# lixinghe1999/VRVQ

Measured on AMD Instinct MI355X. Metric: audio-sec/s encode+RVQ+decode, 44.1 kHz batch-32, 1->8 MI355X; RVQ HBM GB/s, higher is better.
Workload: dtype f32; 1 GPU; DAC_VRVQ VBR 8 cb, level 1.0, 1-s clips, preprocess+encode+decode (z_q_is materialised); model=DAC_VRVQ base (8 cb), global_batch=32, clip_samples=44100, n_codebooks=8, parallelism=dp1 (replicas, no data-path collective)

## Files before the change

include/vrvq.h:

```cpp
#ifndef VRVQ_H_
#define VRVQ_H_

#include <stdint.h>

#ifdef __cplusplus
extern "C" {
#endif

typedef void* vrvq_stream_t;

enum vrvq_status_t {
  VRVQ_OK = 0,
  VRVQ_ERR_ARG = 10001,
  VRVQ_ERR_UNSUPPORTED = 10002
};

enum vrvq_epilogue_t { VRVQ_EPI_NONE = 0, VRVQ_EPI_TANH = 1, VRVQ_EPI_SIGMOID = 2 };

const char* vrvq_status_string(int status);
int vrvq_version(void);


int vrvq_weight_norm(const float* g, const float* v, int rows, int cols, float* w,
                     vrvq_stream_t stream);
// ... 21 lines not shown
                          int dil, int x3, long long* bytes);
int vrvq_conv1d_ws(const float* x, int batch, int cin, int tin, const float* alpha,
                   const float* inv_alpha, const float* w_packed, const uint16_t* w_x3, int cout,
                   int cout_pad, int k, int stride, int pad, int dil, const float* bias,
                   const float* residual, int epilogue, float* y, int tout,
                   const float* alpha_out, const float* inv_alpha_out, float* y_snake,
                   void* workspace, long long ws_bytes, vrvq_stream_t stream);

int vrvq_x3_weight_size(int cin, int k, int cout_pad, long long* n_u16);
int vrvq_pack_x3_weight(const float* w_packed, int cin, int k, int cout_pad, uint16_t* w_x3,
                        vrvq_stream_t stream);

int vrvq_conv1d_proj(const float* x, int batch, int cin, int tin, const float* alpha,
                     const float* inv_alpha, const float* w_packed, const uint16_t* w_x3, int cout,
                     int cout_pad, int k, int pad, int dil, const float* bias, float* y, int tout,
                     const uint16_t* w3in, int nq, float* part, void* workspace,
                     long long ws_bytes, vrvq_stream_t stream);

int vrvq_conv_last_launch(int out[5]);

enum vrvq_plan_kind_t { VRVQ_PLAN_CONV = 0, VRVQ_PLAN_PROJ = 1, VRVQ_PLAN_CONV_TRANSPOSE = 2 };
int vrvq_conv_plan(int kind, int batch, int cin, int tin, int cout, int k, int stride, int pad,
                   int dil, int has_x3, int has_workspace, int out[7]);

int vrvq_pack_conv1d_weight(const float* w, int cout, int cin, int k, int cout_pad,
                            float* w_packed, vrvq_stream_t stream);

int vrvq_residual_unit(const float* x, const float* x_snk, int batch, int channels, int frames,
                       int dil, const float* w7_packed, const uint16_t* w7_x3,
                       const uint16_t* w1_x3, const float* b7,
                       const float* alpha2,
                       const float* inv_alpha2, const float* w1_packed, const float* b1,
                       int cout_pad, float* y, const float* alpha_out,
                       const float* inv_alpha_out, float* y_snake, vrvq_stream_t stream);

int vrvq_conv_transpose1d(const float* x, int batch, int cin, int tin, const float* alpha,
                          const float* inv_alpha, const float* w_packed, int cout,
                          int cout_pad, int stride, const float* bias, float* y,
                          const float* alpha_out, const float* inv_alpha_out, float* y_snake,
                          vrvq_stream_t stream);

int vrvq_conv_transpose1d_pad(const float* x, int batch, int cin, int tin, const float* alpha,
                              const float* inv_alpha, const float* w_packed,
                              const uint16_t* w_x3, int cout,
                              int cout_pad, int stride, int pad, const float* bias, float* y,
                              const float* alpha_out, const float* inv_alpha_out,
// ... 235 lines not shown
```

vrvq_amd/_lib.py:

```python
from __future__ import annotations

import ctypes
import os
import threading

LIB_NAME = "libvrvq_hip.so"
LIB_PATH = os.environ.get("VRVQ_LIB") or os.path.join(os.path.dirname(os.path.abspath(__file__)), LIB_NAME)

_P = ctypes.c_void_p
_I = ctypes.c_int
_F = ctypes.c_float

SIGNATURES = {
    "vrvq_weight_norm": [_P, _P, _I, _I, _P, _P],
    "vrvq_snake_inv_alpha": [_P, _I, _P, _P],
    "vrvq_snake": [_P, _I, _I, _I, _P, _P, _P, _P],
    "vrvq_phase_split": [_P, _I, _I, _I, _I, _I, _I, _P, _P, _P, _P],
    "vrvq_codebook_prep": [_P, _I, _I, _P, _P, _P],
    "vrvq_conv1d": [_P, _I, _I, _I, _P, _P, _P, _P, _I, _I, _I, _I, _I, _I, _P, _P, _I, _P, _I,
                    _P, _P, _P, _P],
    "vrvq_conv1d_workspace": [_I, _I, _I, _I, _I, _I, _I, _I, _I, _P],
    "vrvq_conv1d_ws": [_P, _I, _I, _I, _P, _P, _P, _P, _I, _I, _I, _I, _I, _I, _P, _P, _I, _P,
                       _I, _P, _P, _P, _P, ctypes.c_longlong, _P],
    "vrvq_conv1d_proj": [_P, _I, _I, _I, _P, _P, _P, _P, _I, _I, _I, _I, _I, _P, _P, _I, _P, _I,
                         _P, _P, ctypes.c_longlong, _P],
    "vrvq_x3_weight_size": [_I, _I, _I, _P],
    "vrvq_pack_x3_weight": [_P, _I, _I, _I, _P, _P],
    "vrvq_pack_conv1d_weight": [_P, _I, _I, _I, _I, _P, _P],
    "vrvq_residual_unit": [_P, _P, _I, _I, _I, _I, _P, _P, _P, _P, _P, _P, _P, _P, _I, _P, _P,
                           _P, _P, _P],
    "vrvq_conv_transpose1d": [_P, _I, _I, _I, _P, _P, _P, _I, _I, _I, _P, _P, _P, _P, _P, _P],
    "vrvq_conv_transpose1d_pad": [_P, _I, _I, _I, _P, _P, _P, _P, _I, _I, _I, _I, _P, _P, _P, _P,
                                  _P, _P],
    "vrvq_pack_convt1d_weight": [_P, _I, _I, _I, _I, _P, _P],
    "vrvq_rvq_cross_prep": [_P, _P, _P, _I, _I, _I, _P, _P, _P],
    "vrvq_rvq_frag": [_P, _I, _I, _I, _P, _P],
    "vrvq_rvq_workspace": [_I, _I, _I, _P],
    "vrvq_rvq_encode": [_P, _I, _I, _I, _I, _I, _I, _P, _P, _P, _P, _P, _P, _P, _P, _P, _P, _F,
                        _P, _P, _P, _P, _P, _P, _P, ctypes.c_longlong, _P],
    "vrvq_rvq_w_in_planes_size": [_I, _I, _I, _P],
    "vrvq_rvq_pack_w_in": [_P, _I, _I, _I, _P, _P],
    "vrvq_rvq_workspace_part": [_I, _I, _I, _I, _P],
    "vrvq_rvq_encode_part": [_P, _I, _I, _I, _I, _I, _I, _P, _P, _P, _P, _P, _P, _P, _P, _P, _F,
                             _P, _P, _P, _P, _P, _P, _P, ctypes.c_longlong, _P],
    "vrvq_rvq_fused_clips": [_I, _I, _I, _P],
    "vrvq_rvq_project": [_P, _I, _I, _I, _I, _I, _P, _P, _P],
    "vrvq_rvq_chain": [_P, _I, _I, _I, _I, _I, _P, _P, _P, _P, _P, _P, _P, _F, _P, _P, _P, _P, _P,
                       _P],
# ... 44 lines not shown
    "vrvq_conv1d_wgrad": [_P, _I, _I, _I, _P, _P, _P, _I, _I, _P, _P, _I, _I, _I, _I, _I, _P,
                          ctypes.c_longlong, _P, _P],
    "vrvq_snake_backward_workspace": [_I, _I, _I, _P],
    "vrvq_snake_backward": [_P, _P, _P, _P, _I, _I, _I, _P, _P, _P, ctypes.c_longlong, _P],
    "vrvq_bias_grad_workspace": [_I, _I, _I, _P],
    "vrvq_bias_grad": [_P, _I, _I, _I, _P, _P, ctypes.c_longlong, _P],
    "vrvq_act_backward": [_P, _P, ctypes.c_longlong, _I, _P, _P],
    "vrvq_weight_norm_backward": [_P, _P, _P, _I, _I, _P, _P, _P],
    "vrvq_pack_conv1d_flip": [_P, _I, _I, _I, _I, _P, _P],
    "vrvq_mask_ste": [_P, _P, _P, _I, _I, _I, _F, _I, _I, _P, _P],
    "vrvq_mask_ste_backward": [_P, _P, _P, _I, _I, _I, _F, _I, _P, _P],
    "vrvq_rvq_expand_masked": [_P, _I, _I, _I, _I, _I, _P, _P, _P, _P, _P, _P],
    "vrvq_rvq_backward_workspace": [_I, _I, _I, _P],
    "vrvq_rvq_backward": [_P, _P, _P, _P, _P, _P, _P, _P, _I, _I, _I, _I, _I, _I, _P, _P, _P,
                          _P, _P, _P, _P, _P, _P, _P, _P, _P, _P, ctypes.c_longlong, _P],
}
EXTRA = {"vrvq_status_string": ([_I], ctypes.c_char_p), "vrvq_version": ([], _I),
         "vrvq_rvq_path": ([_I], _I), "vrvq_rvq_plan": ([_I] * 5 + [_P], _I),
         "vrvq_rvq_sync_error": ([_P, _P], _I), "vrvq_rvq_timing": ([_I], _I),
         "vrvq_rvq_timing_read": ([_P, _P], _I), "vrvq_rvq_pending_error": ([_P], _I),
         "vrvq_rvq_debug": ([ctypes.c_uint, ctypes.c_uint], _I),
         "vrvq_rvq_debug_capacity": ([_I], _I), "vrvq_conv_last_launch": ([_P], _I),
         "vrvq_conv_plan": ([_I] * 11 + [_P], _I),
         "vrvq_resample_error": ([], ctypes.c_char_p),
         "vrvq_loudness_error": ([], ctypes.c_char_p),
         "vrvq_bitstream_chunk_frames": ([], _I)}

METRICS_CHUNK = 16384
SPECTRAL_TILE_SAMPLES = 8192
RESAMPLE_TILE = 512
LOUDNESS_CHUNK = 256
LOUDNESS_PLAN_LEN = 30
BITSTREAM_CHUNK_FRAMES = 256


def spectral_tile_frames(window: int) -> int:
    return SPECTRAL_TILE_SAMPLES // int(window)

_lock = threading.Lock()
_lib = None


def load() -> ctypes.CDLL:
    global _lib
    if _lib is not None:
        return _lib
# ... 55 lines not shown


def rvq_debug_capacity(clips: int) -> int:
    return int(load().vrvq_rvq_debug_capacity(int(clips)))


def conv_last_launch() -> dict:
    out = (ctypes.c_int * 5)()
    call("vrvq_conv_last_launch", out)
    return dict(zip(("BM", "BN", "KS", "x3", "S"), (int(v) for v in out)))


PLAN_KINDS = {"conv": 0, "proj": 1, "convt": 2}


def conv_plan(kind, batch: int, cin: int, tin: int, cout: int, k: int, stride: int = 1,
              pad: int = 0, dil: int = 1, x3: bool = True, workspace: bool = True) -> dict:
    out = (ctypes.c_int * 7)()
    call("vrvq_conv_plan", PLAN_KINDS.get(kind, kind), batch, cin, tin, cout, k, stride, pad, dil,
         1 if x3 else 0, 1 if workspace else 0, out)
    return dict(zip(("BM", "BN", "KS", "x3", "S", "path", "WM"), (int(v) for v in out)))


def rvq_timing(on: bool) -> bool:
    return bool(load().vrvq_rvq_timing(1 if on else 0))


def rvq_timing_read():
    ms, n = ctypes.c_float(0.0), ctypes.c_int(0)
    call("vrvq_rvq_timing_read", ctypes.byref(ms), ctypes.byref(n))
    return float(ms.value), int(n.value)


RVQ_PLAN_KEYS = ("kind", "F", "P", "n_fb", "wg_per_clip", "lds", "resident", "clips", "launches",
                 "ws_bytes")
RVQ_PLAN_PT, RVQ_PLAN_CHAIN_EXPAND = 0, 1


def rvq_plan(batch: int, frames: int, nq: int, ncode: int = 1024, resident: int = 0) -> dict:
    out = (ctypes.c_longlong * 10)()
    call("vrvq_rvq_plan", batch, frames, nq, ncode, resident, out)
    return dict(zip(RVQ_PLAN_KEYS, (int(v) for v in out)))


RESAMPLE_PLAN_KEYS = ("old", "new", "W", "K", "ntaps", "out_length", "out_length_max",
                      "taps_len")
# ... 52 lines not shown
```

vrvq_amd/csrc/conv_geom.h:

```cpp
#pragma once

namespace vrvq_conv {

constexpr int chunk_ck(int ks, int bm, int bn) {
  const int ck0 = ks == 1 ? 32 : ks <= 3 ? 16 : ks == 4 ? 8 : ks == 7 ? 8
                  : ks == 8 ? 4 : bn > 32 ? 4 : 2;
  return (bm > 128 && ck0 >= 8) ? ck0 / 2 : ck0;
}

constexpr int win_smax(int ks) { return (ks == 4 || ks == 8 || ks == 16) ? ks / 2 : 1; }
constexpr int win_dmax(int ks) { return ks == 7 ? 9 : 1; }
constexpr int win_xw_max(int ks, int bn) {
  return (bn - 1) * win_smax(ks) + (ks - 1) * win_dmax(ks) + 1;
}
constexpr int win_per_row(int ks, int bn) { return (win_xw_max(ks, bn) + 63) / 64; }

constexpr long long conv_lds_bytes(int ks, int bm, int bn, int xwp) {
  const long long ck = chunk_ck(ks, bm, bn);
  return 2 * (ck * ks * bm + ck * xwp) * 4;
}

constexpr int epi_passes(int bm, int bn) {
  const int need = (bm * bn * 4 + 65535) / 65536;
  return need <= 1 ? 1 : need <= 2 ? 2 : need <= 4 ? 4 : 8;
// ... 16 lines not shown
}
constexpr int x3_nc8(int ks, bool pair) { return x3_ck(ks, pair) / 8; }
constexpr int x3_no(int ks, bool pair) { return ks * x3_nc8(ks, pair); }
constexpr int x3_no2(int ks, bool pair) { return (x3_no(ks, pair) + 1) & ~1; }
constexpr int x3_nstep(int ks, bool pair) { return x3_no2(ks, pair) / 2; }

constexpr int x3_xw_max(int ks, int bn) { return (bn - 1) + (ks - 1) * (ks == 7 ? 9 : 1) + 1; }
constexpr int x3_xwp(int xw) { return (xw + 3) & ~3; }

constexpr int x3_stage_w_bytes(int ks, int bm, bool pair) {
  return pair ? 2 * 3 * x3_no(ks, false) * bm * 16 : 3 * x3_no2(ks, false) * bm * 16;
}

constexpr long long x3_lds_bytes(int ks, int bm, int bn, bool pair, int xw, int snake_cin) {
  const long long xb = 3LL * x3_nc8(ks, pair) * x3_xwp(xw) * 16;
  const long long snake = pair ? 2LL * snake_cin * 4 : 0;
  return x3_stages(bm, bn) * (x3_stage_w_bytes(ks, bm, pair) + xb) + snake;
}

constexpr bool x3_offsets_fit(long long tin, long long m_pad) {
  return 32 * tin * 4 <= 0x7fffffffLL && 49 * m_pad * 16 <= 0x7fffffffLL;
}

constexpr int SMALL_BT = 256;
constexpr int SMALL_SC = 16;
constexpr int SMALL_COUT = 8;
constexpr int SMALL_WMAX = 2048;
constexpr int C1_T = 4;
constexpr int C1_W = 12;
constexpr int CI1_T = 4;
constexpr int CI1_CG = 16;

}
```

vrvq_amd/csrc/misc.hip:

```cpp
#include "common.h"

namespace {

__global__ __launch_bounds__(256) void weight_norm_kernel(const float* __restrict__ g,
                                                          const float* __restrict__ v, int cols,
                                                          float* __restrict__ w) {
  __shared__ float part[256];
  const size_t row = blockIdx.x;
  const float* vr = v + row * cols;
  float ss = 0.0f;
  for (int c = threadIdx.x; c < cols; c += 256) ss = fmaf(vr[c], vr[c], ss);
  part[threadIdx.x] = ss;
  __syncthreads();
  for (int h = 128; h >= 1; h >>= 1) {
    if ((int)threadIdx.x < h) part[threadIdx.x] += part[threadIdx.x + h];
    __syncthreads();
  }
  const float scale = g[row] / sqrtf(part[0]);
  for (int c = threadIdx.x; c < cols; c += 256) w[row * cols + c] = vr[c] * scale;
}

__global__ void inv_alpha_kernel(const float* __restrict__ alpha, int n, float* __restrict__ inv) {
  const int i = blockIdx.x * blockDim.x + threadIdx.x;
  if (i < n) inv[i] = 1.0f / (alpha[i] + 1e-9f);
// ... 193 lines not shown
  if (cdim != 8 || ncode > 4096) return VRVQ_ERR_UNSUPPORTED;
  const long long nf = (long long)batch * frames;
  VRVQ_CHECK_ARG((nf + 255) / 256 < 0x7fffffffLL);
  const size_t lds = (size_t)ncode * 9 * sizeof(float);
  if (lds > 64 * 1024) {
    hipError_t e = hipFuncSetAttribute((const void*)rvq_nearest_kernel,
                                       hipFuncAttributeMaxDynamicSharedMemorySize, (int)lds);
    if (e != hipSuccess) return (int)e;
  }
  hipLaunchKernelGGL(rvq_nearest_kernel, dim3((unsigned)((nf + 255) / 256), nq), dim3(256), lds,
                     as_stream(stream), latents, batch, nlat, frames, cbn, c2, ncode, codes, nq);
  return vrvq_launch_status();
}

extern "C" const char* vrvq_status_string(int status) {
  switch (status) {
    case VRVQ_OK: return "ok";
    case VRVQ_ERR_ARG: return "vrvq: invalid argument (null pointer, size or shape mismatch)";
    case VRVQ_ERR_UNSUPPORTED: return "vrvq: shape outside the instantiated kernel set";
    default: return hipGetErrorString((hipError_t)status);
  }
}

extern "C" int vrvq_version(void) { return 111; }

extern "C" int vrvq_weight_norm(const float* g, const float* v, int rows, int cols, float* w,
                                vrvq_stream_t stream) {
  VRVQ_CHECK_ARG(g && v && w && rows > 0 && cols > 0);
  hipLaunchKernelGGL(weight_norm_kernel, dim3(rows), dim3(256), 0, as_stream(stream), g, v, cols, w);
  return vrvq_launch_status();
}

__global__ __launch_bounds__(256) void snake_rows_kernel(const float* __restrict__ x,
                                                         const float* __restrict__ alpha,
                                                         const float* __restrict__ inv_alpha,
                                                         int channels, int frames, int nseg,
                                                         float* __restrict__ y) {
  const int row = blockIdx.x / nseg, seg = blockIdx.x - row * nseg;
  const int c = row % channels;
  const float al = alpha[c], ia = inv_alpha[c];
  const size_t base = (size_t)row * frames;
#pragma unroll
  for (int u = 0; u < 4; ++u) {
    const int t = seg * 1024 + u * 256 + (int)threadIdx.x;
    if (t < frames) y[base + t] = snake_act(x[base + t], al, ia);
  }
}
// ... 118 lines not shown
```

vrvq_amd/csrc/torch_ops.cpp:

```cpp
#include <ATen/core/Tensor.h>
#include <ATen/ops/empty.h>
#include <ATen/ops/empty_like.h>
#include <ATen/ops/zeros.h>
#include <c10/core/DeviceGuard.h>
#include <c10/hip/HIPStream.h>
#include <torch/library.h>

#include <vector>

#include "../../include/vrvq.h"

namespace {

using at::Tensor;
using c10::optional;

void* stream_of(const Tensor& t) {
  return reinterpret_cast<void*>(c10::hip::getCurrentHIPStream(t.device().index()).stream());
}

void check_rc(int rc, const char* fn) {
  TORCH_CHECK(rc == 0, fn, " failed (", rc, "): ", vrvq_status_string(rc));
}

// ... 157 lines not shown
  TORCH_CHECK(alpha.has_value() == inv_alpha.has_value(), "conv1d: snake needs inv_alpha");
  c10::DeviceGuard guard(x.device());
  const int64_t k = w_packed.size(1), cout_pad = w_packed.size(2);
  const int64_t tout = (tin + 2 * pad - dil * (k - 1) - 1) / stride + 1;
  TORCH_CHECK(tout > 0, "conv1d: input too short");
  if (residual.has_value())
    TORCH_CHECK(residual->sizes() == at::IntArrayRef({B, cout, tout}),
                "conv1d: residual shape must equal the output shape");
  auto [y, ys, _u] = out_pair(x, {B, cout, tout}, alpha_out, inv_alpha_out, want_raw);
  const uint16_t* w3 = stride > 1 ? x3_ptr(w_x3, x, cin * stride, 2, cout_pad)
                                  : x3_ptr(w_x3, x, cin, k, cout_pad);
  long long ws_bytes = 0;
  check_rc(vrvq_conv1d_workspace((int)B, (int)cin, (int)tin, (int)cout, (int)k, (int)stride,
                                 (int)pad, (int)dil, w3 != nullptr, &ws_bytes),
           "vrvq_conv1d_workspace");
  Tensor ws = ws_bytes > 0 ? at::empty({(ws_bytes + 3) / 4}, x.options()) : Tensor();
  check_rc(vrvq_conv1d_ws(x.data_ptr<float>(), (int)B, (int)cin, (int)tin, fp(alpha),
                          fp(inv_alpha), w_packed.data_ptr<float>(), w3, (int)cout,
                          (int)cout_pad, (int)k, (int)stride, (int)pad, (int)dil, fp(bias),
                          fp(residual), (int)epilogue, y.numel() ? y.data_ptr<float>() : nullptr,
                          (int)tout, fp(alpha_out), fp(inv_alpha_out), opt_ptr(ys),
                          ws_bytes > 0 ? ws.data_ptr() : nullptr, ws_bytes, stream_of(x)),
           "vrvq_conv1d_ws");
  return {y, ys};
}

std::tuple<Tensor, Tensor> snake_conv_transpose1d(
    const Tensor& x, const Tensor& w_packed, int64_t cout, int64_t stride,
    const optional<Tensor>& bias, const optional<Tensor>& alpha,
    const optional<Tensor>& inv_alpha, const optional<Tensor>& alpha_out,
    const optional<Tensor>& inv_alpha_out, bool want_raw, int64_t pad,
    const optional<Tensor>& w_x3) {
  check_t(x, "x");
  check_on(w_packed, x, "w_packed");
  check_opt(bias, x, "bias");
  check_opt(alpha, x, "alpha");
  check_opt(inv_alpha, x, "inv_alpha");
  TORCH_CHECK(x.dim() == 3, "conv_transpose1d: x must be (B, C, T)");
  const int64_t p = pad < 0 ? (stride + 1) / 2 : pad;
  TORCH_CHECK(p < stride, "conv_transpose1d: padding must be < stride");
  TORCH_CHECK(w_packed.dim() == 3 && w_packed.size(0) == x.size(1) && w_packed.size(1) == 2,
              "conv_transpose1d: w_packed must be (Cin, 2, cout_pad)");
  TORCH_CHECK(alpha.has_value() == inv_alpha.has_value(),
              "conv_transpose1d: snake needs inv_alpha");
  c10::DeviceGuard guard(x.device());
  const int64_t B = x.size(0), cin = x.size(1), tin = x.size(2);
// ... 1195 lines not shown
  Tensor ws = at::empty({ws_doubles}, x.options().dtype(at::kDouble));
  Tensor out = at::empty({items}, x.options().dtype(at::kDouble));
  check_rc(vrvq_loudness(x.data_ptr<float>(), (int)items, (int)nch, L, (int)sample_rate,
                         ws.data_ptr<double>(), out.data_ptr<double>(), stream_of(x)),
           "vrvq_loudness");
  return out;
}

}

TORCH_LIBRARY(vrvq, m) {
  m.def("weight_norm(Tensor g, Tensor v) -> Tensor");
  m.def("snake_inv_alpha(Tensor alpha) -> Tensor");
  m.def("codebook_prep(Tensor cb) -> (Tensor, Tensor)");
  m.def("pack_conv1d_weight(Tensor w) -> Tensor");
  m.def("pack_convt1d_weight(Tensor w, int stride) -> Tensor");
  m.def("pack_x3_weight(Tensor w_packed, int k) -> Tensor");
  m.def(
      "snake_conv1d(Tensor x, Tensor w_packed, int cout, int stride, int pad, int dil, "
      "Tensor? bias, Tensor? alpha, Tensor? inv_alpha, Tensor? residual, int epilogue, "
      "Tensor? alpha_out, Tensor? inv_alpha_out, bool want_raw, Tensor? w_x3=None) "
      "-> (Tensor, Tensor)");
  m.def(
      "snake_conv_transpose1d(Tensor x, Tensor w_packed, int cout, int stride, Tensor? bias, "
      "Tensor? alpha, Tensor? inv_alpha, Tensor? alpha_out, Tensor? inv_alpha_out, "
      "bool want_raw, int pad=-1, Tensor? w_x3=None) -> (Tensor, Tensor)");
  m.def(
      "residual_unit(Tensor x, Tensor x_snk, int dil, Tensor w7, Tensor b7, Tensor alpha2, "
      "Tensor inv_alpha2, Tensor w1, Tensor b1, Tensor? alpha_out, Tensor? inv_alpha_out, "
      "bool want_raw, Tensor? w7_x3=None, Tensor? w1_x3=None) -> (Tensor, Tensor)");
  m.def("rvq_cross_prep(Tensor w_in_t, Tensor w_out, Tensor b_out) -> (Tensor, Tensor)");
  m.def("rvq_frag(Tensor cbn) -> Tensor");
  m.def(
      "rvq_encode(Tensor z, Tensor w_in_t, Tensor b_in, Tensor cb, Tensor cbf, Tensor c2, "
      "Tensor w_out, Tensor b_out, Tensor mcol, Tensor qb, Tensor? imp, float level, "
      "bool want_z_q_is, bool want_mask) -> (Tensor, Tensor, Tensor, Tensor, Tensor, Tensor)");
  m.def("rvq_pack_w_in(Tensor w_in_t) -> Tensor");
  m.def(
      "snake_conv1d_proj(Tensor x, Tensor w_packed, int cout, int pad, int dil, Tensor? bias, "
      "Tensor? alpha, Tensor? inv_alpha, Tensor? w_x3, Tensor w3in, int nq, bool want_z) "
      "-> (Tensor, Tensor)");
  m.def(
      "rvq_encode_part(Tensor part, int frames, Tensor b_in, Tensor cb, Tensor cbf, Tensor c2, "
      "Tensor w_out, Tensor b_out, Tensor mcol, Tensor qb, Tensor? imp, float level, "
      "bool want_z_q_is, bool want_mask) -> (Tensor, Tensor, Tensor, Tensor, Tensor, Tensor)");
  m.def("rvq_check_error(Tensor like, bool sync) -> int");
// ... 67 lines not shown
      "Tensor w_out, Tensor b_out, Tensor mcol, Tensor qb, Tensor mask) "
      "-> (Tensor, Tensor, Tensor, Tensor, Tensor)");
  m.def(
      "rvq_backward(Tensor dz_q, Tensor g_commit, Tensor g_codebook, Tensor z, Tensor zst, "
      "Tensor latents, Tensor codes, Tensor mask, Tensor w_in_t, Tensor w_out, Tensor b_out, "
      "Tensor mcol, Tensor cb) -> (Tensor, Tensor, Tensor, Tensor, Tensor, Tensor, Tensor)");
  m.def(
      "resample(Tensor x, Tensor taps, Tensor first, int old_rate, int width, int out_length) "
      "-> Tensor");
  m.def(
      "resample_adjoint(Tensor dy, Tensor taps, Tensor first, int old_rate, int width, "
      "int length) -> Tensor");
  m.def("loudness(Tensor x, int sample_rate) -> Tensor");
}

#define VRVQ_IMPLS(m) \
  m.impl("weight_norm", &weight_norm); \
  m.impl("snake_inv_alpha", &snake_inv_alpha); \
  m.impl("codebook_prep", &codebook_prep); \
  m.impl("pack_conv1d_weight", &pack_conv1d_weight); \
  m.impl("pack_convt1d_weight", &pack_convt1d_weight); \
  m.impl("pack_x3_weight", &pack_x3_weight); \
  m.impl("snake_conv1d", &snake_conv1d); \
  m.impl("snake_conv_transpose1d", &snake_conv_transpose1d); \
  m.impl("residual_unit", &residual_unit); \
  m.impl("rvq_cross_prep", &rvq_cross_prep); \
  m.impl("rvq_frag", &rvq_frag); \
  m.impl("rvq_encode", &rvq_encode); \
  m.impl("rvq_pack_w_in", &rvq_pack_w_in); \
  m.impl("snake_conv1d_proj", &snake_conv1d_proj); \
  m.impl("rvq_encode_part", &rvq_encode_part); \
  m.impl("rvq_check_error", &rvq_check_error); \
  m.impl("rvq_gather", &rvq_gather); \
  m.impl("rvq_nearest", &rvq_nearest); \
  m.impl("rvq_expand", &rvq_expand); \
  m.impl("masked_loss", &masked_loss); \
  m.impl("scale_imp", &scale_imp); \
  m.impl("imp_mask", &imp_mask); \
  m.impl("masked_sum", &masked_sum); \
  m.impl("bpf", &bpf); \
  m.impl("rate_curve", &rate_curve); \
  m.impl("rate_solve", &rate_solve); \
  m.impl("scale_imp_rows", &scale_imp_rows); \
  m.impl("rate_solve_capped", &rate_solve_capped); \
  m.impl("scale_imp_packets", &scale_imp_packets); \
  m.impl("signal_metrics", &signal_metrics); \
// ... 28 lines not shown
```

vrvq_amd/layers.py:

```python
from __future__ import annotations

import math
from typing import Optional

import torch
import torch.nn as nn

from . import ops


def _param_key(*ps):
    return tuple((p.device, p.data_ptr(), p._version) for p in ps)


class Snake1d(nn.Module):

    def __init__(self, channels: int):
        super().__init__()
        self.channels = channels
        self.alpha = nn.Parameter(torch.ones(1, channels, 1))
        self._cache = None

    def prepared(self):
        key = _param_key(self.alpha)
# ... 161 lines not shown
            x = x[..., pad:-pad].contiguous()
        return self.block[3](y, snake=self.block[2], residual=x)

    def runs_fused(self) -> bool:
        C = self.block[1].in_channels
        return self.fused and C in ops.RU_FUSED_CHANNELS and not (C == 256 and ops.X3 and
                                                                 ops.RU256_SPLIT)

    def run(self, x: torch.Tensor, x_snk: torch.Tensor, out_snake: Snake1d, want_raw: bool):
        if self.runs_fused():
            w7, cp7 = self.block[1].prepared()
            w1, cp1 = self.block[3].prepared()
            a2, ia2 = self.block[2].prepared()
            return ops.residual_unit(x, x_snk, self.block[1].dilation[0], w7,
                                     self.block[1].bias.detach(), a2, ia2, w1,
                                     self.block[3].bias.detach(), cp7,
                                     out_snake=out_snake.prepared(), want_raw=want_raw,
                                     w7_x3=self.block[1].prepared_x3(),
                                     w1_x3=self.block[3].prepared_x3())
        return self.run_two_launch(x, x_snk, out_snake, want_raw)

    def run_two_launch(self, x, x_snk, out_snake: Snake1d, want_raw: bool):
        _, h_snk = self.block[1](x_snk, out_snake=self.block[2], want_raw=False)
        return self.block[3](h_snk, residual=x, out_snake=out_snake, want_raw=want_raw)


class EncoderBlock(nn.Module):

    def __init__(self, dim: int = 16, stride: int = 1):
        super().__init__()
        self.block = nn.Sequential(
            ResidualUnit(dim // 2, dilation=1),
            ResidualUnit(dim // 2, dilation=3),
            ResidualUnit(dim // 2, dilation=9),
            Snake1d(dim // 2),
            WNConv1d(dim // 2, dim, kernel_size=2 * stride, stride=stride,
                     padding=math.ceil(stride / 2)),
        )

    def forward(self, x):
        for i in range(3):
            x = self.block[i](x)
        return self.block[4](x, snake=self.block[3])

    def entry_snake(self) -> Snake1d:
        return self.block[0].block[0]

# ... 38 lines not shown
```

vrvq_amd/ops.py:

```python
from __future__ import annotations

import os
import threading
from typing import Optional, Tuple

import torch

EPI_NONE, EPI_TANH, EPI_SIGMOID = 0, 1, 2

_HERE = os.path.dirname(os.path.abspath(__file__))
TORCH_LIB_PATH = os.environ.get("VRVQ_TORCH_LIB") or os.path.join(_HERE, "libvrvq_torch.so")
_lock = threading.Lock()
_loaded = False


def load_ops():
    global _loaded
    if _loaded:
        return torch.ops.vrvq
    with _lock:
        if not _loaded:
            if not os.path.exists(TORCH_LIB_PATH):
                raise RuntimeError(
                    f"vrvq_amd: operator library {TORCH_LIB_PATH} is missing; build it with "
# ... 46 lines not shown
    return wp, wp.shape[2]


def pack_convt1d_weight(w: torch.Tensor, stride: int) -> Tuple[torch.Tensor, int]:
    wp = _ops().pack_convt1d_weight(w, int(stride))
    return wp, wp.shape[2]


def conv1d(x: torch.Tensor, w_packed: torch.Tensor, cout: int, cout_pad: int, k: int,
           stride: int = 1, pad: int = 0, dil: int = 1, bias: Optional[torch.Tensor] = None,
           alpha: Optional[torch.Tensor] = None, inv_alpha: Optional[torch.Tensor] = None,
           residual: Optional[torch.Tensor] = None, epilogue: int = EPI_NONE,
           out_snake: Optional[Tuple[torch.Tensor, torch.Tensor]] = None, want_raw: bool = True,
           w_x3: Optional[torch.Tensor] = None):
    if w_packed.dim() != 3 or w_packed.shape[1] != k or w_packed.shape[2] != cout_pad:
        raise RuntimeError("conv1d: w_packed must be (Cin, k, cout_pad)")
    ao, io = out_snake if out_snake is not None else (None, None)
    y, ys = _ops().snake_conv1d(x, w_packed, int(cout), int(stride), int(pad), int(dil), bias,
                                alpha, inv_alpha, residual, int(epilogue), ao, io, bool(want_raw),
                                w_x3)
    return _none(y) if out_snake is None else (_none(y), ys)


def conv1d_proj(x: torch.Tensor, w_packed: torch.Tensor, cout: int, k: int, w3in: torch.Tensor,
                nq: int, pad: int = 0, dil: int = 1, bias: Optional[torch.Tensor] = None,
                alpha: Optional[torch.Tensor] = None, inv_alpha: Optional[torch.Tensor] = None,
                w_x3: Optional[torch.Tensor] = None, want_z: bool = False):
    if w_packed.dim() != 3 or w_packed.shape[1] != k:
        raise RuntimeError("conv1d_proj: w_packed must be (Cin, k, cout_pad)")
    part, z = _ops().snake_conv1d_proj(x, w_packed, int(cout), int(pad), int(dil), bias, alpha,
                                       inv_alpha, w_x3, w3in, int(nq), bool(want_z))
    return part, _none(z)


def conv_transpose1d(x: torch.Tensor, w_packed: torch.Tensor, cout: int, cout_pad: int,
                     stride: int, bias: Optional[torch.Tensor] = None,
                     alpha: Optional[torch.Tensor] = None,
                     inv_alpha: Optional[torch.Tensor] = None,
                     out_snake: Optional[Tuple[torch.Tensor, torch.Tensor]] = None,
                     want_raw: bool = True, pad: int = -1,
                     w_x3: Optional[torch.Tensor] = None):
    ao, io = out_snake if out_snake is not None else (None, None)
    y, ys = _ops().snake_conv_transpose1d(x, w_packed, int(cout), int(stride), bias, alpha,
                                          inv_alpha, ao, io, bool(want_raw), int(pad), w_x3)
    return _none(y) if out_snake is None else (_none(y), ys)

# ... 247 lines not shown

    @reg("vrvq::pack_x3_weight")
    def _(w_packed, k):
        cin, _k, cout_pad = w_packed.shape
        return torch.empty(x3_size(cin, k, cout_pad), dtype=torch.int16, device=w_packed.device)

    @reg("vrvq::pack_convt1d_weight")
    def _(w, stride):
        cin, cout, _k = w.shape
        return f32(w, (cin, 2, round_up(cout * stride, 128 if 128 % stride == 0 else 192)))

    def pair(x, shape, ao, want_raw):
        ys = f32(x, shape) if ao is not None else none(x)
        y = f32(x, shape) if (want_raw or ao is None) else none(x)
        return y, ys

    @reg("vrvq::snake_conv1d")
    def _(x, w_packed, cout, stride, pad, dil, bias, alpha, inv_alpha, residual, epilogue,
          alpha_out, inv_alpha_out, want_raw, w_x3=None):
        B, _c, tin = x.shape
        tout = conv_out_len(tin, w_packed.shape[1], stride, pad, dil)
        return pair(x, (B, cout, tout), alpha_out, want_raw)

    @reg("vrvq::snake_conv_transpose1d")
    def _(x, w_packed, cout, stride, bias, alpha, inv_alpha, alpha_out, inv_alpha_out, want_raw,
          pad=-1, w_x3=None):
        B, _c, tin = x.shape
        tout = convt_out_len(tin, stride, pad)
        return pair(x, (B, cout, tout), alpha_out, want_raw)

    @reg("vrvq::residual_unit")
    def _(x, x_snk, dil, w7, b7, alpha2, inv_alpha2, w1, b1, alpha_out, inv_alpha_out, want_raw,
          w7_x3=None, w1_x3=None):
        return pair(x, tuple(x.shape), alpha_out, want_raw)

    @reg("vrvq::rvq_cross_prep")
    def _(w_in_t, w_out, b_out):
        nq, _D, d = w_in_t.shape
        return f32(w_in_t, (nq, nq, d, d)), f32(w_in_t, (nq, d))

    @reg("vrvq::rvq_frag")
    def _(cbn):
        return torch.empty_like(cbn)

    @reg("vrvq::rvq_encode")
    def _(z, w_in_t, b_in, cb, cbf, c2, w_out, b_out, mcol, qb, imp, level, want_z_q_is,
# ... 219 lines not shown
```

Baseline: 806.6 audio-sec/s.

## Add specialized k=1 conv kernel with fused residual and snake for residual units

Adds a dedicated pointwise (k=1) convolution kernel for the residual-unit second conv. It stages the whole input-channel slice in LDS as three bf16 split planes, runs the x3 bf16 MFMA accumulation with double-buffered weight loads, and fuses bias, residual add and the output snake into the epilogue. Residual loads are issued early to overlap with staging. It replaces the generic conv path in run_two_launch when the channel count is 192/256/384, falling back otherwise. It costs extra code paths and large LDS use, which may reduce occupancy.

New measurement: 811.8 audio-sec/s, median of 6. Within noise of the previous version (+0.6%).

```diff
diff --git a/include/vrvq.h b/include/vrvq.h
--- a/include/vrvq.h
+++ b/include/vrvq.h
@@ -67,6 +67,12 @@
 enum vrvq_plan_kind_t { VRVQ_PLAN_CONV = 0, VRVQ_PLAN_PROJ = 1, VRVQ_PLAN_CONV_TRANSPOSE = 2 };
 int vrvq_conv_plan(int kind, int batch, int cin, int tin, int cout, int k, int stride, int pad,
                    int dil, int has_x3, int has_workspace, int out[7]);
+
+int vrvq_conv1d_k1_skip(const float* x, int batch, int cin, int tin, const uint16_t* w_x3,
+                        int cout, int cout_pad, const float* bias, const float* residual,
+                        float* y, const float* alpha_out, const float* inv_alpha_out,
+                        float* y_snake, vrvq_stream_t stream);
+int vrvq_conv1d_k1_skip_plan(int batch, int cin, int tin, int cout, int out[5]);
 
 int vrvq_pack_conv1d_weight(const float* w, int cout, int cin, int k, int cout_pad,
                             float* w_packed, vrvq_stream_t stream);
diff --git a/vrvq_amd/_lib.py b/vrvq_amd/_lib.py
--- a/vrvq_amd/_lib.py
+++ b/vrvq_amd/_lib.py
@@ -24,6 +24,7 @@
                        _I, _P, _P, _P, _P, ctypes.c_longlong, _P],
     "vrvq_conv1d_proj": [_P, _I, _I, _I, _P, _P, _P, _P, _I, _I, _I, _I, _I, _P, _P, _I, _P, _I,
                          _P, _P, ctypes.c_longlong, _P],
+    "vrvq_conv1d_k1_skip": [_P, _I, _I, _I, _P, _I, _I, _P, _P, _P, _P, _P, _P, _P],
     "vrvq_x3_weight_size": [_I, _I, _I, _P],
     "vrvq_pack_x3_weight": [_P, _I, _I, _I, _P, _P],
     "vrvq_pack_conv1d_weight": [_P, _I, _I, _I, _I, _P, _P],
@@ -114,6 +115,7 @@
          "vrvq_rvq_debug": ([ctypes.c_uint, ctypes.c_uint], _I),
          "vrvq_rvq_debug_capacity": ([_I], _I), "vrvq_conv_last_launch": ([_P], _I),
          "vrvq_conv_plan": ([_I] * 11 + [_P], _I),
+         "vrvq_conv1d_k1_skip_plan": ([_I] * 4 + [_P], _I),
          "vrvq_resample_error": ([], ctypes.c_char_p),
          "vrvq_loudness_error": ([], ctypes.c_char_p),
          "vrvq_bitstream_chunk_frames": ([], _I)}
@@ -215,6 +217,24 @@
     return dict(zip(("BM", "BN", "KS", "x3", "S", "path", "WM"), (int(v) for v in out)))
 
 
+K1_SKIP_PLAN_KEYS = ("BM", "BN", "threads", "lds", "grid")
+ERR_UNSUPPORTED = 10002
+
+
+def k1_skip_plan(batch: int, channels: int, frames: int, cout: int = 0):
+    out = (ctypes.c_int * 5)()
+    lib = load()
+    rc = lib.vrvq_conv1d_k1_skip_plan(int(batch), int(channels), int(frames),
+                                      int(cout or channels), out)
+    if rc == ERR_UNSUPPORTED:
+        return None
+    if rc != 0:
+        msg = lib.vrvq_status_string(rc)
+        raise RuntimeError(f"vrvq_conv1d_k1_skip_plan failed ({rc}): "
+                           f"{msg.decode() if msg else 'unknown'}")
+    return dict(zip(K1_SKIP_PLAN_KEYS, (int(v) for v in out)))
+
+
 def rvq_timing(on: bool) -> bool:
     return bool(load().vrvq_rvq_timing(1 if on else 0))
 
diff --git a/vrvq_amd/csrc/conv_geom.h b/vrvq_amd/csrc/conv_geom.h
--- a/vrvq_amd/csrc/conv_geom.h
+++ b/vrvq_amd/csrc/conv_geom.h
@@ -62,6 +62,23 @@
   return 32 * tin * 4 <= 0x7fffffffLL && 49 * m_pad * 16 <= 0x7fffffffLL;
 }
 
+struct K1sTile {
+  int BM, BN, WM, NW, WPE;
+};
+constexpr K1sTile k1s_tile(int c) {
+  return c == 192 ? K1sTile{192, 64, 2, 4, 2}
+       : c == 256 ? K1sTile{256, 64, 4, 8, 2}
+       : c == 384 ? K1sTile{384, 64, 4, 8, 2}
+                  : K1sTile{0, 0, 0, 0, 0};
+}
+constexpr long long k1s_lds_bytes(int c, int bn) { return 6LL * c * bn; }
+constexpr long long k1s_lds_total(int c, int bm, int bn) { return k1s_lds_bytes(c, bn) + 3LL * bm * 4; }
+constexpr bool k1s_offsets_fit(long long c, long long tin) { return c * tin * 4 <= 0x7fffffffLL; }
+constexpr long long k1s_grid(int c, long long batch, long long tin) {
+  const K1sTile t = k1s_tile(c);
+  return t.BM == 0 ? 0 : batch * ((tin + t.BN - 1) / t.BN) * (c / t.BM);
+}
+
 constexpr int SMALL_BT = 256;
 constexpr int SMALL_SC = 16;
 constexpr int SMALL_COUT = 8;
diff --git a/vrvq_amd/csrc/conv_k1_skip.hip b/vrvq_amd/csrc/conv_k1_skip.hip
--- /dev/null
+++ b/vrvq_amd/csrc/conv_k1_skip.hip
@@ -0,0 +1,271 @@
+#include "common.h"
+#include "conv_core.h"
+#include "conv_x3.h"
+
+namespace {
+
+using namespace vrvq_conv;
+
+struct K1sArgs {
+  const float* x;
+  const u32x4* w3;
+  const float* bias;
+  const float* res;
+  float* y;
+  const float* alpha_o;
+  const float* inv_alpha_o;
+  float* ys;
+  int tin, m_pad, n_nt;
+};
+
+typedef float f32x4u __attribute__((ext_vector_type(4), aligned(4)));
+
+template <int C, int BM, int BN, int WM, int NW, int WPE>
+__global__ __launch_bounds__(64 * NW) __attribute__((amdgpu_waves_per_eu(WPE, WPE)))
+void k1_skip_kernel(K1sArgs a) {
+  using TC = TileCfg<BM, BN, WM, NW>;
+  constexpr int NT = TC::NT, RM = TC::RM, RN = TC::RN, TM = TC::TM, TN = TC::TN;
+  constexpr int NC8 = C / 8;
+  constexpr int NQ = C / 16;
+  constexpr int N_MT = C / BM;
+  constexpr int XI = NC8 * BN / NT;
+  constexpr int NV = BN / 4;
+  constexpr int ITER = BM * NV / NT;
+  static_assert(C % 32 == 0 && C % BM == 0, "whole k = 1 chunks, whole row tiles");
+  static_assert((NC8 * BN) % NT == 0 && NT % BN == 0, "staging: whole items, one column per thread");
+  static_assert((BM * NV) % NT == 0 && NT % NV == 0, "epilogue: whole items, one column group per thread");
+  static_assert(RM >= 1 && RN >= 1 && TM % 32 == 0 && TN % 32 == 0 && NQ % 2 == 0, "tile");
+  extern __shared__ __attribute__((aligned(16))) float smem[];
+
+  int blk = blockIdx.x;
+  const int m0 = (blk % N_MT) * BM;
+  blk /= N_MT;
+  const int nt = blk % a.n_nt, b = blk / a.n_nt;
+  const int n0 = nt * BN;
+  const int T = a.tin;
+  const int tid = threadIdx.x, lane = tid & 63, wave = tid >> 6;
+  const int wm = wave % WM, wn = wave / WM;
+  const int lr = lane & 31, lh = lane >> 5;
+
+  float* tab = reinterpret_cast<float*>(reinterpret_cast<char*>(smem) + k1s_lds_bytes(C, BN));
+  for (int r = tid; r < BM; r += NT) {
+    tab[r] = a.bias ? a.bias[m0 + r] : 0.0f;
+    tab[BM + r] = a.ys ? a.alpha_o[m0 + r] : 0.0f;
+    tab[2 * BM + r] = a.ys ? a.inv_alpha_o[m0 + r] : 0.0f;
+  }
+
+  const int ncols = min(BN, T - n0);
+  const int nl = (tid % NV) * 4;
+  const bool inrow = nl + 4 <= ncols;
+  f32x4u rs[ITER];
+  {
+    const float* xb = a.x + (size_t)b * C * T;
+    const int col = tid % BN, t = n0 + col;
+    const unsigned xo = ((unsigned)((tid / BN) * 8) * (unsigned)T + (unsigned)min(t, T - 1)) * 4u;
+    float xr[XI][8];
+#pragma unroll
+    for (int it = 0; it < XI; ++it)
+#pragma unroll
+      for (int u = 0; u < 8; ++u) {
+        const float* xu = xb + (size_t)(it * (NT / BN) * 8 + u) * T;
+        xr[it][u] = *reinterpret_cast<const float*>(reinterpret_cast<const char*>(xu) + xo);
+      }
+    __builtin_amdgcn_sched_barrier(0);
+    {
+      const float* resb = a.res + (size_t)b * C * T;
+      const unsigned ro = inrow ? ((unsigned)(m0 + tid / NV) * (unsigned)T + (unsigned)(n0 + nl)) * 4u : 0u;
+      const unsigned rstep = inrow ? (unsigned)(NT / NV) * (unsigned)T * 4u : 0u;
+#pragma unroll
+      for (int it = 0; it < ITER; ++it)
+        rs[it] = *reinterpret_cast<const f32x4u*>(reinterpret_cast<const char*>(resb) + (ro + it * rstep));
+    }
+    __builtin_amdgcn_sched_barrier(0);
+    u32x4* xs = reinterpret_cast<u32x4*>(smem);
+    const bool ok = t < T;
+#pragma unroll
+    for (int it = 0; it < XI; ++it) {
+      float v[8];
+#pragma unroll
+      for (int u = 0; u < 8; ++u) v[u] = ok ? xr[it][u] : 0.0f;
+      unsigned h[4], m[4], l[4];
+#pragma unroll
+      for (int u = 0; u < 4; ++u) split3x2(v[2 * u], v[2 * u + 1], h[u], m[u], l[u]);
+      const int e = tid + it * NT;
+      xs[0 * NC8 * BN + e] = u32x4{h[0], h[1], h[2], h[3]};
+      xs[1 * NC8 * BN + e] = u32x4{m[0], m[1], m[2], m[3]};
+      xs[2 * NC8 * BN + e] = u32x4{l[0], l[1], l[2], l[3]};
+    }
+  }
+  __syncthreads();
+
+  f32x16 acc[RM][RN];
+#pragma unroll
+  for (int i = 0; i < RM; ++i)
+#pragma unroll
+    for (int j = 0; j < RN; ++j)
+#pragma unroll
+      for (int r = 0; r < 16; ++r) acc[i][j][r] = 0.0f;
+
+  const u32x4* hs = reinterpret_cast<const u32x4*>(smem);
+  const unsigned wlo = ((unsigned)lh * (unsigned)a.m_pad + (unsigned)(m0 + wm * TM + lr)) * 16u;
+  auto lda = [&](int q, u32x4 (&av)[3][RM]) {
+    const u32x4* wq = a.w3 + (size_t)((q >> 1) * 12 + 2 * (q & 1)) * a.m_pad;
+    const unsigned wl = x3_opaque(wlo);
+#pragma unroll
+    for (int p = 0; p < 3; ++p)
+#pragma unroll
+      for (int i = 0; i < RM; ++i)
+        av[p][i] = *reinterpret_cast<const u32x4*>(
+            reinterpret_cast<const char*>(wq + (size_t)(p * 4) * a.m_pad + i * 32) + wl);
+  };
+  auto step = [&](int q, const u32x4 (&av)[3][RM]) {
+    u32x4 bv[3][RN];
+    const int o = 2 * q + lh;
+#pragma unroll
+    for (int p = 0; p < 3; ++p)
+#pragma unroll
+      for (int j = 0; j < RN; ++j) bv[p][j] = hs[((size_t)p * NC8 + o) * BN + wn * TN + j * 32 + lr];
+#pragma unroll
+    for (int i = 0; i < RM; ++i)
+#pragma unroll
+      for (int j = 0; j < RN; ++j) {
+        f32x16 t = acc[i][j];
+        t = mfma_bf16(av[1][i], bv[1][j], t);
+        t = mfma_bf16(av[0][i], bv[2][j], t);
+        t = mfma_bf16(av[2][i], bv[0][j], t);
+        t = mfma_bf16(av[0][i], bv[1][j], t);
+        t = mfma_bf16(av[1][i], bv[0][j], t);
+        acc[i][j] = mfma_bf16(av[0][i], bv[0][j], t);
+      }
+  };
+  u32x4 a0[3][RM], a1[3][RM];
+  lda(0, a0);
+#pragma unroll 1
+  for (int q = 0; q < NQ; q += 2) {
+    lda(q + 1, a1);
+    __builtin_amdgcn_sched_barrier(0);
+    step(q, a0);
+    __builtin_amdgcn_sched_barrier(0);
+    lda(min(q + 2, NQ - 1), a0);
+    __builtin_amdgcn_sched_barrier(0);
+    step(q + 1, a1);
+    __builtin_amdgcn_sched_barrier(0);
+  }
+  __syncthreads();
+
+  float* ct = smem;
+#pragma unroll
+  for (int i = 0; i < RM; ++i)
+#pragma unroll
+    for (int j = 0; j < RN; ++j)
+#pragma unroll
+      for (int r = 0; r < 16; ++r)
+        ct[(wm * TM + i * 32 + (r & 3) + 8 * (r >> 2) + 4 * lh) * BN + wn * TN + j * 32 + lr] =
+            acc[i][j][r];
+  __syncthreads();
+  if (ncols == BN && (T & 3) == 0) {
+#pragma unroll
+    for (int it = 0; it < ITER; ++it) {
+      const int ml = tid / NV + it * (NT / NV);
+      const float4 c = *reinterpret_cast<const float4*>(ct + ml * BN + nl);
+      const float bb = tab[ml];
+      float v[4] = {c.x + bb, c.y + bb, c.z + bb, c.w + bb};
+#pragma unroll
+      for (int q = 0; q < 4; ++q) v[q] = rs[it][q] + v[q];
+      const size_t ob = ((size_t)b * C + m0 + ml) * T + n0 + nl;
+      if (a.y) *reinterpret_cast<float4*>(a.y + ob) = make_float4(v[0], v[1], v[2], v[3]);
+      if (a.ys) {
+        snake_n1<4>(v, tab[BM + ml], tab[2 * BM + ml]);
+        *reinterpret_cast<float4*>(a.ys + ob) = make_float4(v[0], v[1], v[2], v[3]);
+      }
+    }
+    return;
+  }
+  if (nl >= ncols) return;
+#pragma unroll 1
+  for (int it = 0; it < ITER; ++it) {
+    const int ml = tid / NV + it * (NT / NV);
+    const float4 c = *reinterpret_cast<const float4*>(ct + ml * BN + nl);
+    const float bb = tab[ml];
+    float v[4] = {c.x + bb, c.y + bb, c.z + bb, c.w + bb};
+    const size_t ob = ((size_t)b * C + m0 + ml) * T + n0 + nl;
+#pragma unroll
+    for (int q = 0; q < 4; ++q)
+      if (nl + q < ncols) v[q] = a.res[ob + q] + v[q];
+    if (a.y) {
+#pragma unroll
+      for (int q = 0; q < 4; ++q)
+        if (nl + q < ncols) a.y[ob + q] = v[q];
+    }
+    if (a.ys) {
+      snake_n1<4>(v, tab[BM + ml], tab[2 * BM + ml]);
+#pragma unroll
+      for (int q = 0; q < 4; ++q)
+        if (nl + q < ncols) a.ys[ob + q] = v[q];
+    }
+  }
+}
+
+template <int C>
+int launch_k1s(K1sArgs a, int batch, hipStream_t st) {
+  constexpr K1sTile t = k1s_tile(C);
+  static_assert(t.BM > 0, "no tile for this C");
+  constexpr int lds = (int)k1s_lds_total(C, t.BM, t.BN);
+  static_assert(lds <= 160 * 1024, "planes fit in LDS");
+  auto kernel = k1_skip_kernel<C, t.BM, t.BN, t.WM, t.NW, t.WPE>;
+  const long long grid = k1s_grid(C, batch, a.tin);
+  if (grid <= 0 || grid > 0x7fffffffLL) return VRVQ_ERR_ARG;
+  a.n_nt = (a.tin + t.BN - 1) / t.BN;
+  if (lds > 64 * 1024) {
+    hipError_t e = hipFuncSetAttribute((const void*)kernel,
+                                       hipFuncAttributeMaxDynamicSharedMemorySize, lds);
+    if (e != hipSuccess) return (int)e;
+  }
+  hipLaunchKernelGGL(kernel, dim3((unsigned)grid), dim3(64 * t.NW), lds, st, a);
+  return vrvq_launch_status();
+}
+
+bool k1s_geometry_ok(int batch, int cin, int tin, int cout, int cout_pad) {
+  return batch > 0 && cin > 0 && tin > 0 && cout > 0 && cout_pad >= cout && cout_pad % 128 == 0;
+}
+
+}
+
+extern "C" int vrvq_conv1d_k1_skip(const float* x, int batch, int cin, int tin,
+                                   const uint16_t* w_x3, int cout, int cout_pad,
+                                   const float* bias, const float* residual, float* y,
+                                   const float* alpha_out, const float* inv_alpha_out,
+                                   float* y_snake, vrvq_stream_t stream) {
+  VRVQ_CHECK_ARG(x && (y || y_snake));
+  VRVQ_CHECK_ARG(y_snake == nullptr || (alpha_out && inv_alpha_out));
+  VRVQ_CHECK_ARG(k1s_geometry_ok(batch, cin, tin, cout, cout_pad));
+  if (w_x3 == nullptr || residual == nullptr || cin != cout || k1s_tile(cin).BM == 0)
+    return VRVQ_ERR_UNSUPPORTED;
+  if (!x3_offsets_fit(tin, cout_pad) || !k1s_offsets_fit(cin, tin)) return VRVQ_ERR_UNSUPPORTED;
+  K1sArgs a{};
+  a.x = x; a.w3 = reinterpret_cast<const u32x4*>(w_x3); a.bias = bias; a.res = residual; a.y = y;
+  a.alpha_o = alpha_out; a.inv_alpha_o = inv_alpha_out; a.ys = y_snake;
+  a.tin = tin; a.m_pad = cout_pad;
+  hipStream_t st = as_stream(stream);
+  switch (cin) {
+    case 192: return launch_k1s<192>(a, batch, st);
+    case 256: return launch_k1s<256>(a, batch, st);
+    case 384: return launch_k1s<384>(a, batch, st);
+    default: return VRVQ_ERR_UNSUPPORTED;
+  }
+}
+
+extern "C" int vrvq_conv1d_k1_skip_plan(int batch, int cin, int tin, int cout, int out[5]) {
+  VRVQ_CHECK_ARG(out);
+  const long long cout_pad = ((long long)cout + 127) / 128 * 128;
+  VRVQ_CHECK_ARG(cout > 0 && cout < 0x7fffff00 && k1s_geometry_ok(batch, cin, tin, cout, (int)cout_pad));
+  const K1sTile t = k1s_tile(cin);
+  if (cin != cout || t.BM == 0) return VRVQ_ERR_UNSUPPORTED;
+  if (!x3_offsets_fit(tin, cout_pad) || !k1s_offsets_fit(cin, tin)) return VRVQ_ERR_UNSUPPORTED;
+  const long long grid = k1s_grid(cin, batch, tin);
+  if (grid <= 0 || grid > 0x7fffffffLL) return VRVQ_ERR_ARG;
+  out[0] = t.BM; out[1] = t.BN; out[2] = 64 * t.NW;
+  out[3] = (int)k1s_lds_total(cin, t.BM, t.BN);
+  out[4] = (int)grid;
+  return 0;
+}
diff --git a/vrvq_amd/csrc/misc.hip b/vrvq_amd/csrc/misc.hip
--- a/vrvq_amd/csrc/misc.hip
+++ b/vrvq_amd/csrc/misc.hip
@@ -239,7 +239,7 @@
   }
 }
 
-extern "C" int vrvq_version(void) { return 111; }
+extern "C" int vrvq_version(void) { return 112; }
 
 extern "C" int vrvq_weight_norm(const float* g, const float* v, int rows, int cols, float* w,
                                 vrvq_stream_t stream) {
diff --git a/vrvq_amd/csrc/torch_ops.cpp b/vrvq_amd/csrc/torch_ops.cpp
--- a/vrvq_amd/csrc/torch_ops.cpp
+++ b/vrvq_amd/csrc/torch_ops.cpp
@@ -203,6 +203,28 @@
                           (int)tout, fp(alpha_out), fp(inv_alpha_out), opt_ptr(ys),
                           ws_bytes > 0 ? ws.data_ptr() : nullptr, ws_bytes, stream_of(x)),
            "vrvq_conv1d_ws");
+  return {y, ys};
+}
+
+std::tuple<Tensor, Tensor> conv1d_k1_skip(const Tensor& x, const Tensor& w_x3, int64_t cout_pad,
+                                          const optional<Tensor>& bias, const Tensor& residual,
+                                          const optional<Tensor>& alpha_out,
+                                          const optional<Tensor>& inv_alpha_out, bool want_raw) {
+  check_t(x, "x");
+  check_opt(bias, x, "bias");
+  check_on(residual, x, "residual");
+  TORCH_CHECK(x.dim() == 3 && residual.sizes() == x.sizes(),
+              "conv1d_k1_skip: residual must have the shape of x (B, C, T)");
+  c10::DeviceGuard guard(x.device());
+  const int64_t B = x.size(0), C = x.size(1), T = x.size(2);
+  TORCH_CHECK(!bias.has_value() || bias->numel() == C, "conv1d_k1_skip: one bias per channel");
+  auto [y, ys, _u] = out_pair(x, {B, C, T}, alpha_out, inv_alpha_out, want_raw);
+  const optional<Tensor> w3(w_x3);
+  check_rc(vrvq_conv1d_k1_skip(x.data_ptr<float>(), (int)B, (int)C, (int)T,
+                               x3_ptr(w3, x, C, 1, cout_pad), (int)C, (int)cout_pad, fp(bias),
+                               residual.data_ptr<float>(), opt_ptr(y), fp(alpha_out),
+                               fp(inv_alpha_out), opt_ptr(ys), stream_of(x)),
+           "vrvq_conv1d_k1_skip");
   return {y, ys};
 }
 
@@ -1444,6 +1466,9 @@
       "Tensor? alpha_out, Tensor? inv_alpha_out, bool want_raw, Tensor? w_x3=None) "
       "-> (Tensor, Tensor)");
   m.def(
+      "conv1d_k1_skip(Tensor x, Tensor w_x3, int cout_pad, Tensor? bias, Tensor residual, "
+      "Tensor? alpha_out, Tensor? inv_alpha_out, bool want_raw) -> (Tensor, Tensor)");
+  m.def(
       "snake_conv_transpose1d(Tensor x, Tensor w_packed, int cout, int stride, Tensor? bias, "
       "Tensor? alpha, Tensor? inv_alpha, Tensor? alpha_out, Tensor? inv_alpha_out, "
       "bool want_raw, int pad=-1, Tensor? w_x3=None) -> (Tensor, Tensor)");
@@ -1557,6 +1582,7 @@
   m.impl("pack_convt1d_weight", &pack_convt1d_weight); \
   m.impl("pack_x3_weight", &pack_x3_weight); \
   m.impl("snake_conv1d", &snake_conv1d); \
+  m.impl("conv1d_k1_skip", &conv1d_k1_skip); \
   m.impl("snake_conv_transpose1d", &snake_conv_transpose1d); \
   m.impl("residual_unit", &residual_unit); \
   m.impl("rvq_cross_prep", &rvq_cross_prep); \
diff --git a/vrvq_amd/layers.py b/vrvq_amd/layers.py
--- a/vrvq_amd/layers.py
+++ b/vrvq_amd/layers.py
@@ -207,7 +207,11 @@
 
     def run_two_launch(self, x, x_snk, out_snake: Snake1d, want_raw: bool):
         _, h_snk = self.block[1](x_snk, out_snake=self.block[2], want_raw=False)
-        return self.block[3](h_snk, residual=x, out_snake=out_snake, want_raw=want_raw)
+        c1 = self.block[3]
+        wp, cout_pad = c1.prepared()
+        return ops.conv1d_k1_skip(h_snk, wp, c1.out_channels, cout_pad, c1.bias.detach(), x,
+                                  out_snake=out_snake.prepared(), want_raw=want_raw,
+                                  w_x3=c1.prepared_x3())
 
 
 class EncoderBlock(nn.Module):
diff --git a/vrvq_amd/ops.py b/vrvq_amd/ops.py
--- a/vrvq_amd/ops.py
+++ b/vrvq_amd/ops.py
@@ -92,6 +92,31 @@
     return _none(y) if out_snake is None else (_none(y), ys)
 
 
+_K1_SKIP_PLANS = {}
+
+
+def k1_skip_supported(batch: int, channels: int, frames: int) -> bool:
+    key = (int(batch), int(channels), int(frames))
+    if key not in _K1_SKIP_PLANS:
+        from . import _lib
+        _K1_SKIP_PLANS[key] = _lib.k1_skip_plan(*key)
+    return _K1_SKIP_PLANS[key] is not None
+
+
+def conv1d_k1_skip(x: torch.Tensor, w_packed: torch.Tensor, cout: int, cout_pad: int,
+                   bias: Optional[torch.Tensor], residual: torch.Tensor,
+                   out_snake: Optional[Tuple[torch.Tensor, torch.Tensor]] = None,
+                   want_raw: bool = True, w_x3: Optional[torch.Tensor] = None):
+    B, C, T = x.shape
+    if (w_x3 is None or residual is None or C != cout or x.device.type != "cuda"
+            or not k1_skip_supported(B, C, T)):
+        return conv1d(x, w_packed, cout, cout_pad, 1, bias=bias, residual=residual,
+                      out_snake=out_snake, want_raw=want_raw, w_x3=w_x3)
+    ao, io = out_snake if out_snake is not None else (None, None)
+    y, ys = _ops().conv1d_k1_skip(x, w_x3, int(cout_pad), bias, residual, ao, io, bool(want_raw))
+    return _none(y) if out_snake is None else (_none(y), ys)
+
+
 def conv1d_proj(x: torch.Tensor, w_packed: torch.Tensor, cout: int, k: int, w3in: torch.Tensor,
                 nq: int, pad: int = 0, dil: int = 1, bias: Optional[torch.Tensor] = None,
                 alpha: Optional[torch.Tensor] = None, inv_alpha: Optional[torch.Tensor] = None,
@@ -385,6 +410,10 @@
         tout = conv_out_len(tin, w_packed.shape[1], stride, pad, dil)
         return pair(x, (B, cout, tout), alpha_out, want_raw)
 
+    @reg("vrvq::conv1d_k1_skip")
+    def _(x, w_x3, cout_pad, bias, residual, alpha_out, inv_alpha_out, want_raw):
+        return pair(x, tuple(x.shape), alpha_out, want_raw)
+
     @reg("vrvq::snake_conv_transpose1d")
     def _(x, w_packed, cout, stride, bias, alpha, inv_alpha, alpha_out, inv_alpha_out, want_raw,
           pad=-1, w_x3=None):
```
